# nyuolab/OmniBioTE

Hardware: AMD Instinct MI355X
Metric: MLM train tokens/sec, small (8L/1024d) ctx=1024 at 1/2/4/8 MI355X (higher is better)
Workload: dtype bf16

## Files before the change

omnibiote_amd/csrc/elementwise.hip:

```cpp
#include "common.h"
#include <stdlib.h>

namespace {

template <bool INVERSE>
__global__ __launch_bounds__(256) void rope_kernel(bf16* __restrict__ qkv, const float* __restrict__ cos_t,
                                                    const float* __restrict__ sin_t, int64_t rows, int64_t T, int C, int hs) {
    const int chunks_per_row = 2 * C / 8;
    const int64_t total = rows * chunks_per_row;
    for (int64_t i = (int64_t)blockIdx.x * blockDim.x + threadIdx.x; i < total; i += (int64_t)gridDim.x * blockDim.x) {
        const int64_t row = i / chunks_per_row;
        const int col = (int)(i % chunks_per_row) * 8;
        const int d = col % hs;
        const int64_t t = row % T;
        bf16* ptr = qkv + row * 3 * C + col;
        const bf16x8 v = *reinterpret_cast<const bf16x8*>(ptr);
        const f32x4 c = *reinterpret_cast<const f32x4*>(cos_t + t * (hs / 2) + d / 2);
        const f32x4 s = *reinterpret_cast<const f32x4*>(sin_t + t * (hs / 2) + d / 2);
        bf16x8 o;
#pragma unroll
        for (int j = 0; j < 4; ++j) {
            const float xe = bf2f(v[2 * j]), xo = bf2f(v[2 * j + 1]);
            const float sj = INVERSE ? -s[j] : s[j];
            o[2 * j] = f2bf(xe * c[j] - xo * sj);
            o[2 * j + 1] = f2bf(xe * sj + xo * c[j]);
        }
        *reinterpret_cast<bf16x8*>(ptr) = o;
    }
}

__device__ __forceinline__ int64_t clamp_tok(int64_t tok, int64_t vocab) { return tok < 0 ? 0 : (tok >= vocab ? vocab - 1 : tok); }

__global__ __launch_bounds__(256) void embed_fwd_kernel(const int64_t* __restrict__ idx, const bf16* __restrict__ wte,
                                                         bf16* __restrict__ out, int64_t rows, int cols, int64_t vocab, DropCfg dc) {
    const int cpr = cols / 8;
    const int64_t total = rows * cpr;
    for (int64_t i = (int64_t)blockIdx.x * blockDim.x + threadIdx.x; i < total; i += (int64_t)gridDim.x * blockDim.x) {
        const int64_t r = i / cpr;
        const int c = (int)(i % cpr) * 8;
        const int64_t tok = clamp_tok(idx[r], vocab);
        bf16x8 v = *reinterpret_cast<const bf16x8*>(wte + tok * cols + c);
        if (dc.thresh16) {
            const uint32_t rk = drop_rowkey((uint64_t)r, dc);
#pragma unroll
            for (int jj = 0; jj < 4; ++jj) {
                const uint32_t bits = drop_pair_bits(rk, (uint32_t)(c >> 1) + jj);
#pragma unroll
                for (int e = 0; e < 2; ++e) v[2 * jj + e] = drop_keep_bits(bits, (uint32_t)e, dc) ? f2bf(bf2f(v[2 * jj + e]) * dc.scale) : f2bf(0.f);
            }
        }
        *reinterpret_cast<bf16x8*>(out + r * cols + c) = v;
    }
}

__global__ __launch_bounds__(256) void dropout_kernel(const bf16* in, bf16* out, int64_t n8, int64_t cols, DropCfg dc) {
    for (int64_t i = (int64_t)blockIdx.x * blockDim.x + threadIdx.x; i < n8; i += (int64_t)gridDim.x * blockDim.x) {
        bf16x8 v = reinterpret_cast<const bf16x8*>(in)[i];
        const int64_t row = (i * 8) / cols;
        const uint32_t c = (uint32_t)((i * 8) - row * cols);
        const uint32_t rk = drop_rowkey((uint64_t)row, dc);
        for (int jj = 0; jj < 4; ++jj) {
            const uint32_t bits = drop_pair_bits(rk, (c >> 1) + jj);
#pragma unroll
            for (int e = 0; e < 2; ++e) v[2 * jj + e] = drop_keep_bits(bits, (uint32_t)e, dc) ? f2bf(bf2f(v[2 * jj + e]) * dc.scale) : f2bf(0.f);
        }
        reinterpret_cast<bf16x8*>(out)[i] = v;
    }
}

constexpr int EMB_CHUNK = 32;

template <bool ACC>
__device__ __forceinline__ void embed_store_row(bf16* dst, const float (&acc)[8]) {
    bf16x8 o;
#pragma unroll
    for (int j = 0; j < 8; ++j) o[j] = f2bf(acc[j]);
    if (ACC) {
        const bf16x8 old = *reinterpret_cast<const bf16x8*>(dst);
#pragma unroll
        for (int j = 0; j < 8; ++j) o[j] = f2bf(bf2f(old[j]) + bf2f(o[j]));
    }
    *reinterpret_cast<bf16x8*>(dst) = o;
}
template <bool ACC>
__device__ __forceinline__ void embed_store_row(float* dst, const float (&acc)[8]) {
    f32x4 lo = f32x4{acc[0], acc[1], acc[2], acc[3]}, hi = f32x4{acc[4], acc[5], acc[6], acc[7]};
    if (ACC) {
        lo += *reinterpret_cast<const f32x4*>(dst);
        hi += *reinterpret_cast<const f32x4*>(dst + 4);
    }
    *reinterpret_cast<f32x4*>(dst) = lo;
    *reinterpret_cast<f32x4*>(dst + 4) = hi;
}

template <bool ACC, class DST = bf16>
__global__ __launch_bounds__(128) void embed_bwd_chunk_kernel(const int64_t* __restrict__ idx, const int32_t* __restrict__ order,
                                                               const bf16* __restrict__ dout, DST* __restrict__ dwte,
                                                               float* __restrict__ slab, int64_t rows, int cols, int64_t vocab, DropCfg dc) {
    __shared__ int32_t s_row[EMB_CHUNK];
    __shared__ int64_t s_tok[EMB_CHUNK + 2];
    const int64_t c = blockIdx.x;
    const int64_t p0 = c * EMB_CHUNK;
    const int n = (int)((rows - p0) < EMB_CHUNK ? (rows - p0) : EMB_CHUNK);
    if (threadIdx.x < n) {
        const int32_t r = order[p0 + threadIdx.x];
        s_row[threadIdx.x] = r;
        s_tok[threadIdx.x + 1] = clamp_tok(idx[r], vocab);
    }
    if (threadIdx.x == 64) s_tok[0] = p0 > 0 ? clamp_tok(idx[order[p0 - 1]], vocab) : -1;
    if (threadIdx.x == 65) s_tok[n + 1] = (p0 + n < rows) ? clamp_tok(idx[order[p0 + n]], vocab) : -1;
    __syncthreads();
    const bool left_open = s_tok[0] == s_tok[1];
    const bool right_open = s_tok[n + 1] == s_tok[n];
    for (int col = threadIdx.x * 8; col < cols; col += 128 * 8) {
        float acc[8];
#pragma unroll
        for (int j = 0; j < 8; ++j) acc[j] = 0.f;
        int seg_start = 0;
        for (int i = 0; i < n; ++i) {
            const bf16x8 v = *reinterpret_cast<const bf16x8*>(dout + (int64_t)s_row[i] * cols + col);
            if (dc.thresh16) {
                const uint32_t rk = drop_rowkey((uint64_t)s_row[i], dc);
                for (int jj = 0; jj < 4; ++jj) {
                    const uint32_t bits = drop_pair_bits(rk, (uint32_t)(col >> 1) + jj);
#pragma unroll
                    for (int e = 0; e < 2; ++e)
                        if (drop_keep_bits(bits, (uint32_t)e, dc)) acc[2 * jj + e] += bf2f(f2bf(bf2f(v[2 * jj + e]) * dc.scale));
                }
            } else {
#pragma unroll
                for (int j = 0; j < 8; ++j) acc[j] += bf2f(v[j]);
            }
            const bool seg_end = (i == n - 1) || (s_tok[i + 2] != s_tok[i + 1]);
            if (seg_end) {
                const bool is_first = seg_start == 0, is_last = i == n - 1;
                if ((is_first && left_open) || (is_last && right_open)) {
                    float* dst = slab + ((c * 2 + (is_first ? 0 : 1)) * cols + col);
                    *reinterpret_cast<f32x4*>(dst) = f32x4{acc[0], acc[1], acc[2], acc[3]};
                    *reinterpret_cast<f32x4*>(dst + 4) = f32x4{acc[4], acc[5], acc[6], acc[7]};
                } else {
                    embed_store_row<ACC>(dwte + s_tok[i + 1] * cols + col, acc);
                }
#pragma unroll
                for (int j = 0; j < 8; ++j) acc[j] = 0.f;
                seg_start = i + 1;
            }
        }
    }
}

template <bool ACC, class DST = bf16>
__global__ __launch_bounds__(128) void embed_bwd_span_kernel(const int64_t* __restrict__ idx, const int32_t* __restrict__ order,
                                                              DST* __restrict__ dwte, const float* __restrict__ slab,
                                                              int64_t rows, int cols, int64_t nchunks, int64_t vocab) {
    const int64_t c = blockIdx.x;
    const int64_t p0 = c * EMB_CHUNK;
    const int64_t p1 = (p0 + EMB_CHUNK < rows) ? p0 + EMB_CHUNK : rows;
    const int64_t first = clamp_tok(idx[order[p0]], vocab), last = clamp_tok(idx[order[p1 - 1]], vocab);
    const bool single = first == last;
    const bool left_open = p0 > 0 && clamp_tok(idx[order[p0 - 1]], vocab) == first;
    const bool right_open = p1 < rows && clamp_tok(idx[order[p1]], vocab) == last;
    if (!right_open || (single && left_open)) return;
    const int slot0 = single ? 0 : 1;
    for (int col = threadIdx.x * 8; col < cols; col += 128 * 8) {
        float acc[8];
        const float* src = slab + ((c * 2 + slot0) * cols + col);
#pragma unroll
        for (int j = 0; j < 8; ++j) acc[j] = src[j];
        for (int64_t cc = c + 1; cc < nchunks; ++cc) {
            const int64_t q0 = cc * EMB_CHUNK;
            const int64_t q1 = (q0 + EMB_CHUNK < rows) ? q0 + EMB_CHUNK : rows;
            if (clamp_tok(idx[order[q0]], vocab) != last) break;
            const float* s2 = slab + ((cc * 2) * cols + col);
#pragma unroll
            for (int j = 0; j < 8; ++j) acc[j] += s2[j];
            if (clamp_tok(idx[order[q1 - 1]], vocab) != last) break;
        }
        embed_store_row<ACC>(dwte + last * cols + col, acc);
    }
}

__global__ __launch_bounds__(256) void acc32_add_kernel(float* __restrict__ acc32, const bf16* __restrict__ src, bf16* __restrict__ out,
                                                         int64_t n8, int mode) {
    for (int64_t i = (int64_t)blockIdx.x * 256 + threadIdx.x; i < n8; i += (int64_t)gridDim.x * 256) {
        float v[8];
        if (src) {
            const bf16x8 sv = *reinterpret_cast<const bf16x8*>(src + i * 8);
#pragma unroll
            for (int j = 0; j < 8; ++j) v[j] = bf2f(sv[j]);
        } else {
#pragma unroll
            for (int j = 0; j < 8; ++j) v[j] = 0.f;
        }
        if (mode != OBTE_ACC32_FIRST) {
            const f32x4 lo = *reinterpret_cast<const f32x4*>(acc32 + i * 8), hi = *reinterpret_cast<const f32x4*>(acc32 + i * 8 + 4);
#pragma unroll
            for (int j = 0; j < 4; ++j) { v[j] += lo[j]; v[4 + j] += hi[j]; }
        }
        if (src || mode == OBTE_ACC32_FIRST) {
            *reinterpret_cast<f32x4*>(acc32 + i * 8) = f32x4{v[0], v[1], v[2], v[3]};
            *reinterpret_cast<f32x4*>(acc32 + i * 8 + 4) = f32x4{v[4], v[5], v[6], v[7]};
        }
        if (mode == OBTE_ACC32_LAST) {
            bf16x8 o;
#pragma unroll
            for (int j = 0; j < 8; ++j) o[j] = f2bf(v[j]);
            *reinterpret_cast<bf16x8*>(out + i * 8) = o;
        }
    }
}

__global__ __launch_bounds__(256) void masked_ce_kernel(const bf16* __restrict__ logits, const int64_t* __restrict__ target,
                                                         const uint8_t* __restrict__ mlm_mask, const uint8_t* __restrict__ prev_mask,
                                                         const float* __restrict__ grad_scale, float row_scale,
                                                         float* __restrict__ row_loss, bf16* __restrict__ dlogits, int64_t vocab,
                                                         const int64_t* __restrict__ row_index, const float* __restrict__ row_scale_vec) {
    __shared__ float red[8];
    const int64_t r = blockIdx.x;
    const int64_t src = row_index ? row_index[r] : r;
    const int lane = threadIdx.x & 63, wave = threadIdx.x >> 6;
    bf16* drow = dlogits + r * vocab;
    if (!row_index && mlm_mask && !mlm_mask[r]) {
        if (threadIdx.x == 0 && row_loss) row_loss[r] = 0.f;
        if (prev_mask && !prev_mask[r]) return;
        const bf16x8 z = {};
        for (int64_t c = (int64_t)threadIdx.x * 8; c < vocab; c += 256 * 8) *reinterpret_cast<bf16x8*>(drow + c) = z;
        return;
    }
    const bf16* lrow = logits + src * vocab;
    float m = -INFINITY, l = 0.f;
    for (int64_t c = (int64_t)threadIdx.x * 8; c < vocab; c += 256 * 8) {
        const bf16x8 v = *reinterpret_cast<const bf16x8*>(lrow + c);
        float mx = bf2f(v[0]);
#pragma unroll
        for (int j = 1; j < 8; ++j) mx = fmaxf(mx, bf2f(v[j]));
        const float mn = fmaxf(m, mx);
        float add = 0.f;
#pragma unroll
        for (int j = 0; j < 8; ++j) add += __expf(bf2f(v[j]) - mn);
        l = l * __expf(m - mn) + add;
        m = mn;
    }
    const float wm = wave_max(m);
    l = wave_sum(m == -INFINITY ? 0.f : l * __expf(m - wm));
    if (lane == 0) { red[wave] = wm; red[4 + wave] = l; }
    __syncthreads();
    const float bm = fmaxf(fmaxf(red[0], red[1]), fmaxf(red[2], red[3]));
    const float bl = red[4] * __expf(red[0] - bm) + red[5] * __expf(red[1] - bm) + red[6] * __expf(red[2] - bm) + red[7] * __expf(red[3] - bm);
    const float lse = bm + __logf(bl);
    int64_t tgt = target[src];
    tgt = tgt < 0 ? 0 : (tgt >= vocab ? vocab - 1 : tgt);
    const float rsc = row_scale_vec ? row_scale * row_scale_vec[r] : row_scale;
    if (threadIdx.x == 0 && row_loss) row_loss[r] = (lse - bf2f(lrow[tgt])) * rsc;
    const float gs = grad_scale ? rsc * grad_scale[0] : rsc;
    for (int64_t c = (int64_t)threadIdx.x * 8; c < vocab; c += 256 * 8) {
        const bf16x8 v = *reinterpret_cast<const bf16x8*>(lrow + c);
        bf16x8 o;
#pragma unroll
        for (int j = 0; j < 8; ++j) {
            float p = __expf(bf2f(v[j]) - lse);
            if (c + j == tgt) p -= 1.0f;
            o[j] = f2bf(p * gs);
        }
        *reinterpret_cast<bf16x8*>(drow + c) = o;
    }
}

template <int NCH>
__global__ __launch_bounds__(256, 2) void masked_ce_regs_kernel(const bf16* __restrict__ logits, const int64_t* __restrict__ target,
                                                              const float* __restrict__ grad_scale, float row_scale,
                                                              float* __restrict__ row_loss, bf16* __restrict__ dlogits, int64_t vocab,
                                                              const int64_t* __restrict__ row_index, const float* __restrict__ row_scale_vec) {
    __shared__ float red[8];
    const int64_t r = blockIdx.x;
    const int64_t src = row_index ? row_index[r] : r;
    const int lane = threadIdx.x & 63, wave = threadIdx.x >> 6;
    bf16* drow = dlogits + r * vocab;
    const bf16* lrow = logits + src * vocab;
    bf16x8 v[NCH];
#pragma unroll
    for (int i = 0; i < NCH; ++i) {
        const int64_t c = ((int64_t)i * 256 + threadIdx.x) * 8;
        v[i] = bf16x8{};
        if (c < vocab) v[i] = *reinterpret_cast<const bf16x8*>(lrow + c);
    }
    float m = -INFINITY, l = 0.f;
#pragma unroll
    for (int i = 0; i < NCH; ++i) {
        const int64_t c = ((int64_t)i * 256 + threadIdx.x) * 8;
        if (c < vocab) {
            float mx = bf2f(v[i][0]);
#pragma unroll
            for (int j = 1; j < 8; ++j) mx = fmaxf(mx, bf2f(v[i][j]));
            const float mn = fmaxf(m, mx);
            float add = 0.f;
#pragma unroll
            for (int j = 0; j < 8; ++j) add += __expf(bf2f(v[i][j]) - mn);
            l = l * __expf(m - mn) + add;
            m = mn;
        }
    }
    const float wm = wave_max(m);
    l = wave_sum(m == -INFINITY ? 0.f : l * __expf(m - wm));
    if (lane == 0) { red[wave] = wm; red[4 + wave] = l; }
    __syncthreads();
    const float bm = fmaxf(fmaxf(red[0], red[1]), fmaxf(red[2], red[3]));
    const float bl = red[4] * __expf(red[0] - bm) + red[5] * __expf(red[1] - bm) + red[6] * __expf(red[2] - bm) + red[7] * __expf(red[3] - bm);
    const float lse = bm + __logf(bl);
    int64_t tgt = target[src];
    tgt = tgt < 0 ? 0 : (tgt >= vocab ? vocab - 1 : tgt);
    const float rsc = row_scale_vec ? row_scale * row_scale_vec[r] : row_scale;
    if (threadIdx.x == 0 && row_loss) row_loss[r] = (lse - bf2f(lrow[tgt])) * rsc;
    const float gs = grad_scale ? rsc * grad_scale[0] : rsc;
#pragma unroll
    for (int i = 0; i < NCH; ++i) {
        const int64_t c = ((int64_t)i * 256 + threadIdx.x) * 8;
        if (c < vocab) {
            bf16x8 o;
#pragma unroll
            for (int j = 0; j < 8; ++j) {
                float p = __expf(bf2f(v[i][j]) - lse);
                if (c + j == tgt) p -= 1.0f;
                o[j] = f2bf(p * gs);
            }
            *reinterpret_cast<bf16x8*>(drow + c) = o;
        }
    }
}

template <int NCH, bool NT>
__global__ __launch_bounds__(256, 1) void masked_ce_pipe_kernel(const bf16* __restrict__ logits, const int64_t* __restrict__ target,
                                                                 const float* __restrict__ grad_scale, float row_scale,
// ... 255 lines not shown
        }
        bf16x8 pp;
#pragma unroll
        for (int j = 0; j < 8; ++j) {
            const int h = j >> 2, k = j & 3;
            const float gj = bf2f(gg[j]) * cc;
            float pj = ww[h][k] * decay;
            const float m0 = mm[h][k];
            const float mj = __builtin_fmaf(w1, gj - m0, m0);
            float vj = vv[h][k] * b2;
            const float wg = w2 * gj;
            vj = __builtin_fmaf(wg, gj, vj);
            float d = sqrtf(vj);
            d = d / bc2s;
            d = d + eps;
            const float num = neg_step * mj;
            const float upd = num / d;
            pj = pj + upd;
            ww[h][k] = pj; mm[h][k] = mj; vv[h][k] = vj;
            pp[j] = f2bf(pj);
        }
        *reinterpret_cast<bf16x8*>(p + i) = pp;
#pragma unroll
        for (int h = 0; h < 2; ++h) {
            *reinterpret_cast<f32x4*>(w + i + 4 * h) = ww[h];
            *reinterpret_cast<f32x4*>(m + i + 4 * h) = mm[h];
            *reinterpret_cast<f32x4*>(v + i + 4 * h) = vv[h];
        }
    }
}

__global__ __launch_bounds__(256) void sumsq_multi_partials_kernel(MtTable t, float* __restrict__ partials) {
    __shared__ float red[4];
    const int ti = mt_find(t, blockIdx.x);
    const int64_t base = (int64_t)(blockIdx.x - t.first[ti]) * MT_CHUNK;
    const int64_t end = min(base + (int64_t)MT_CHUNK, t.n[ti]);
    const bf16* g = t.g[ti];
    float s = 0.f;
    for (int64_t i = base + threadIdx.x * 8; i < end; i += 256 * 8) {
        const bf16x8 v = *reinterpret_cast<const bf16x8*>(g + i);
#pragma unroll
        for (int j = 0; j < 8; ++j) { const float f = bf2f(v[j]); s += f * f; }
    }
    s = wave_sum(s);
    if ((threadIdx.x & 63) == 0) red[threadIdx.x >> 6] = s;
    __syncthreads();
    if (threadIdx.x == 0) partials[blockIdx.x] = ((red[0] + red[1]) + red[2]) + red[3];
}

__global__ __launch_bounds__(256) void clip_coef_kernel(const float* __restrict__ partials, int64_t n, float max_norm, float* __restrict__ out) {
    __shared__ double red[256];
    double s = 0.0;
    for (int64_t i = threadIdx.x; i < n; i += 256) s += (double)partials[i];
    red[threadIdx.x] = s;
    __syncthreads();
#pragma unroll
    for (int o = 128; o > 0; o >>= 1) {
        if ((int)threadIdx.x < o) red[threadIdx.x] += red[threadIdx.x + o];
        __syncthreads();
    }
    if (threadIdx.x == 0) {
        const float norm_sq = (float)red[0];
        out[0] = norm_sq;
        out[1] = fminf(1.0f, (1.0f / (sqrtf(norm_sq) + 1e-6f)) * max_norm);
    }
}

inline unsigned stream_grid(int64_t work_items, int per_block) {
    int64_t b = cdiv64(work_items, per_block);
    return (unsigned)(b < 1 ? 1 : (b > 2048 ? 2048 : b));
}

}

extern "C" int obte_rope_qk_inplace(obte_bf16* qkv, const float* cos_t, const float* sin_t, int64_t B, int64_t T,
                                    int n_head, int head_dim, int inverse, obte_stream s) {
    OBTE_REQUIRE(qkv && cos_t && sin_t, "obte_rope_qk_inplace: null pointer");
    OBTE_REQUIRE_ALIGNED("obte_rope_qk_inplace", qkv, "qkv", 16);
    OBTE_REQUIRE_ALIGNED("obte_rope_qk_inplace", cos_t, "cos_t", 16);
    OBTE_REQUIRE_ALIGNED("obte_rope_qk_inplace", sin_t, "sin_t", 16);
    OBTE_REQUIRE(B > 0 && T > 0 && n_head > 0 && head_dim % 8 == 0, "obte_rope_qk_inplace: head_dim must be a multiple of 8");
    const int C = n_head * head_dim;
    const int64_t rows = B * T, total = rows * (2 * C / 8);
    hipStream_t st = (hipStream_t)s;
    if (inverse)
        hipLaunchKernelGGL((rope_kernel<true>), dim3(stream_grid(total, 256)), dim3(256), 0, st, (bf16*)qkv, cos_t, sin_t, rows, T, C, head_dim);
    else
        hipLaunchKernelGGL((rope_kernel<false>), dim3(stream_grid(total, 256)), dim3(256), 0, st, (bf16*)qkv, cos_t, sin_t, rows, T, C, head_dim);
    OBTE_CHECK_LAUNCH("obte_rope_qk_inplace");
    return OBTE_OK;
}

static int check_p(const char* who, float p) {
    OBTE_REQUIRE(p >= 0.f && p < 1.f, "%s: dropout p must be in [0, 1) (got %g)", who, (double)p);
    return OBTE_OK;
}

extern "C" int obte_embedding_fwd_dropout(const int64_t* idx, const obte_bf16* wte, obte_bf16* out, int64_t rows, int cols,
                                          int64_t vocab, float p, uint64_t seed, obte_stream s) {
    OBTE_REQUIRE(idx && wte && out, "obte_embedding_fwd: null pointer");
    OBTE_REQUIRE_ALIGNED("obte_embedding_fwd", wte, "wte", 16);
    OBTE_REQUIRE_ALIGNED("obte_embedding_fwd", out, "out", 16);
    OBTE_REQUIRE(rows >= 0 && cols > 0 && cols % 8 == 0 && vocab > 0, "obte_embedding_fwd: cols must be a multiple of 8");
    if (check_p("obte_embedding_fwd", p)) return OBTE_EINVAL;
    if (rows == 0) return OBTE_OK;
    hipLaunchKernelGGL(embed_fwd_kernel, dim3(stream_grid(rows * (cols / 8), 256)), dim3(256), 0, (hipStream_t)s, idx,
                       (const bf16*)wte, (bf16*)out, rows, cols, vocab, make_drop(p, seed, OBTE_SITE_EMBED));
    OBTE_CHECK_LAUNCH("obte_embedding_fwd");
    return OBTE_OK;
}

extern "C" int obte_embedding_fwd(const int64_t* idx, const obte_bf16* wte, obte_bf16* out, int64_t rows, int cols,
                                  int64_t vocab, obte_stream s) {
    return obte_embedding_fwd_dropout(idx, wte, out, rows, cols, vocab, 0.f, 0, s);
}

__global__ __launch_bounds__(256) void dropout_rows_kernel(const bf16* __restrict__ in, const bf16* __restrict__ aux, bf16* __restrict__ out,
                                                           const int64_t* __restrict__ rows, int64_t n_rows, int cols, DropCfg cfg) {
    const int64_t i = (int64_t)blockIdx.x * 4 + (threadIdx.x >> 6);
    if (i >= n_rows) return;
    const int lane = threadIdx.x & 63;
    const uint32_t rk = drop_rowkey((uint64_t)rows[i], cfg);
    for (int c = lane * 8; c < cols; c += 512) {
        bf16x8 v = *reinterpret_cast<const bf16x8*>(in + i * cols + c);
        bf16x8 a = {};
        if (aux) a = *reinterpret_cast<const bf16x8*>(aux + i * cols + c);
#pragma unroll
        for (int jj = 0; jj < 4; ++jj) {
            const uint32_t bits = drop_pair_bits(rk, ((uint32_t)c >> 1) + jj);
#pragma unroll
            for (int e = 0; e < 2; ++e) {
                const int j = 2 * jj + e;
                const float t = drop_keep_bits(bits, (uint32_t)e, cfg) ? bf2f(f2bf(bf2f(v[j]) * cfg.scale)) : 0.f;
                v[j] = aux ? f2bf(bf2f(a[j]) + t) : f2bf(t);
            }
        }
        *reinterpret_cast<bf16x8*>(out + i * cols + c) = v;
    }
}

extern "C" int obte_dropout_bf16(const obte_bf16* in, obte_bf16* out, int64_t n, int64_t cols, float p, uint64_t seed, int32_t site,
                                 obte_stream s) {
    OBTE_REQUIRE_ALIGNED("obte_dropout_bf16", in, "in", 16);
    OBTE_REQUIRE_ALIGNED("obte_dropout_bf16", out, "out", 16);
    OBTE_REQUIRE(in && out && n > 0 && n % 8 == 0, "obte_dropout_bf16: null pointer or n not a positive multiple of 8");
    OBTE_REQUIRE(cols > 0 && cols % 8 == 0 && n % cols == 0 && cols < (1ll << 32), "obte_dropout_bf16: cols must be a multiple of 8 that divides n");
    if (check_p("obte_dropout_bf16", p)) return OBTE_EINVAL;
    hipLaunchKernelGGL(dropout_kernel, dim3(stream_grid(n / 8, 256)), dim3(256), 0, (hipStream_t)s, (const bf16*)in, (bf16*)out, n / 8,
                       cols, make_drop(p, seed, (uint32_t)site));
    OBTE_CHECK_LAUNCH("obte_dropout_bf16");
    return OBTE_OK;
}

extern "C" int64_t obte_embedding_bwd_ws_bytes(int64_t rows, int cols) {
    return cdiv64(rows, EMB_CHUNK) * 2 * (int64_t)cols * (int64_t)sizeof(float);
}

extern "C" int obte_embedding_bwd_dropout(const int64_t* idx, const int32_t* order, const obte_bf16* dout, obte_bf16* dwte,
                                          void* ws, int64_t rows, int cols, int64_t vocab, int accumulate, float p, uint64_t seed,
                                          obte_stream s) {
    OBTE_REQUIRE(idx && order && dout && dwte && ws, "obte_embedding_bwd: null pointer");
    OBTE_REQUIRE_ALIGNED("obte_embedding_bwd", dout, "dout", 16);
    OBTE_REQUIRE_ALIGNED("obte_embedding_bwd", dwte, "dwte", 16);
    OBTE_REQUIRE_ALIGNED("obte_embedding_bwd", ws, "ws", 16);
    if (check_p("obte_embedding_bwd", p)) return OBTE_EINVAL;
    const DropCfg dc = make_drop(p, seed, OBTE_SITE_EMBED);
    OBTE_REQUIRE(rows > 0 && cols > 0 && cols % 8 == 0 && vocab > 0, "obte_embedding_bwd: bad shape");
    OBTE_REQUIRE(rows < (1ll << 31), "obte_embedding_bwd: too many rows");
    hipStream_t st = (hipStream_t)s;
    if (!accumulate && hipMemsetAsync(dwte, 0, (size_t)vocab * cols * sizeof(obte_bf16), st) != hipSuccess) {
        obte_set_error("obte_embedding_bwd: memset failed");
        return OBTE_ELAUNCH;
    }
    const int64_t nchunks = cdiv64(rows, EMB_CHUNK);
    if (accumulate)
        hipLaunchKernelGGL(embed_bwd_chunk_kernel<true>, dim3((unsigned)nchunks), dim3(128), 0, st, idx, order, (const bf16*)dout,
                           (bf16*)dwte, (float*)ws, rows, cols, vocab, dc);
    else
        hipLaunchKernelGGL(embed_bwd_chunk_kernel<false>, dim3((unsigned)nchunks), dim3(128), 0, st, idx, order, (const bf16*)dout,
                           (bf16*)dwte, (float*)ws, rows, cols, vocab, dc);
    OBTE_CHECK_LAUNCH("obte_embedding_bwd(chunk)");
    if (accumulate)
        hipLaunchKernelGGL(embed_bwd_span_kernel<true>, dim3((unsigned)nchunks), dim3(128), 0, st, idx, order, (bf16*)dwte,
                           (const float*)ws, rows, cols, nchunks, vocab);
    else
        hipLaunchKernelGGL(embed_bwd_span_kernel<false>, dim3((unsigned)nchunks), dim3(128), 0, st, idx, order, (bf16*)dwte,
                           (const float*)ws, rows, cols, nchunks, vocab);
    OBTE_CHECK_LAUNCH("obte_embedding_bwd(span)");
    return OBTE_OK;
}

extern "C" int obte_acc32_add_bf16(float* acc32, const obte_bf16* src, obte_bf16* out, int64_t n, int mode, obte_stream s) {
    OBTE_REQUIRE_ALIGNED("obte_acc32_add_bf16", acc32, "acc32", 16);
    OBTE_REQUIRE_ALIGNED("obte_acc32_add_bf16", src, "src", 16);
    OBTE_REQUIRE_ALIGNED("obte_acc32_add_bf16", out, "out", 16);
    OBTE_REQUIRE(acc32 && n > 0 && n % 8 == 0, "obte_acc32_add_bf16: null buffer or n not a positive multiple of 8");
    OBTE_REQUIRE(mode >= OBTE_ACC32_FIRST && mode <= OBTE_ACC32_LAST && (mode != OBTE_ACC32_LAST || out), "obte_acc32_add_bf16: bad mode, or LAST without out");
    if (!src && mode == OBTE_ACC32_MORE) return OBTE_OK;
    hipLaunchKernelGGL(acc32_add_kernel, dim3(stream_grid(n / 8, 256)), dim3(256), 0, (hipStream_t)s, acc32, (const bf16*)src, (bf16*)out, n / 8, mode);
    OBTE_CHECK_LAUNCH("obte_acc32_add_bf16");
    return OBTE_OK;
}

extern "C" int obte_embedding_bwd_acc32(const int64_t* idx, const int32_t* order, const obte_bf16* dout, float* acc32, obte_bf16* dwte,
                                        void* ws, int64_t rows, int cols, int64_t vocab, int mode, float p, uint64_t seed, obte_stream s) {
    OBTE_REQUIRE(idx && order && dout && acc32 && ws, "obte_embedding_bwd_acc32: null pointer");
    OBTE_REQUIRE_ALIGNED("obte_embedding_bwd_acc32", dout, "dout", 16);
    OBTE_REQUIRE_ALIGNED("obte_embedding_bwd_acc32", acc32, "acc32", 16);
    OBTE_REQUIRE_ALIGNED("obte_embedding_bwd_acc32", dwte, "dwte", 16);
    OBTE_REQUIRE_ALIGNED("obte_embedding_bwd_acc32", ws, "ws", 16);
    OBTE_REQUIRE(mode >= OBTE_ACC32_FIRST && mode <= OBTE_ACC32_LAST && (mode != OBTE_ACC32_LAST || dwte), "obte_embedding_bwd_acc32: bad mode, or LAST without dwte");
    if (check_p("obte_embedding_bwd_acc32", p)) return OBTE_EINVAL;
    const DropCfg dc = make_drop(p, seed, OBTE_SITE_EMBED);
    OBTE_REQUIRE(rows > 0 && cols > 0 && cols % 8 == 0 && vocab > 0, "obte_embedding_bwd_acc32: bad shape");
    OBTE_REQUIRE(rows < (1ll << 31), "obte_embedding_bwd_acc32: too many rows");
    hipStream_t st = (hipStream_t)s;
    const bool first = mode == OBTE_ACC32_FIRST;
    if (first && hipMemsetAsync(acc32, 0, (size_t)vocab * cols * sizeof(float), st) != hipSuccess) {
        obte_set_error("obte_embedding_bwd_acc32: memset failed");
        return OBTE_ELAUNCH;
    }
    const int64_t nchunks = cdiv64(rows, EMB_CHUNK);
    if (first)
        hipLaunchKernelGGL((embed_bwd_chunk_kernel<false, float>), dim3((unsigned)nchunks), dim3(128), 0, st, idx, order, (const bf16*)dout, acc32, (float*)ws,
                           rows, cols, vocab, dc);
    else
        hipLaunchKernelGGL((embed_bwd_chunk_kernel<true, float>), dim3((unsigned)nchunks), dim3(128), 0, st, idx, order, (const bf16*)dout, acc32, (float*)ws,
                           rows, cols, vocab, dc);
    OBTE_CHECK_LAUNCH("obte_embedding_bwd_acc32(chunk)");
    if (first)
        hipLaunchKernelGGL((embed_bwd_span_kernel<false, float>), dim3((unsigned)nchunks), dim3(128), 0, st, idx, order, acc32, (const float*)ws, rows, cols,
                           nchunks, vocab);
    else
        hipLaunchKernelGGL((embed_bwd_span_kernel<true, float>), dim3((unsigned)nchunks), dim3(128), 0, st, idx, order, acc32, (const float*)ws, rows, cols,
                           nchunks, vocab);
    OBTE_CHECK_LAUNCH("obte_embedding_bwd_acc32(span)");
    if (mode == OBTE_ACC32_LAST) return obte_acc32_add_bf16(acc32, nullptr, dwte, vocab * (int64_t)cols, OBTE_ACC32_LAST, s);
    return OBTE_OK;
}

extern "C" int obte_embedding_bwd_acc(const int64_t* idx, const int32_t* order, const obte_bf16* dout, obte_bf16* dwte,
                                      void* ws, int64_t rows, int cols, int64_t vocab, int accumulate, obte_stream s) {
    return obte_embedding_bwd_dropout(idx, order, dout, dwte, ws, rows, cols, vocab, accumulate, 0.f, 0, s);
}

extern "C" int obte_embedding_bwd(const int64_t* idx, const int32_t* order, const obte_bf16* dout, obte_bf16* dwte,
                                  void* ws, int64_t rows, int cols, int64_t vocab, obte_stream s) {
    return obte_embedding_bwd_dropout(idx, order, dout, dwte, ws, rows, cols, vocab, 0, 0.f, 0, s);
}

extern "C" int obte_masked_ce_fwd_bwd_reuse(const obte_bf16* logits, const int64_t* target, const uint8_t* mlm_mask,
                                            const uint8_t* prev_mask, const float* grad_scale, float row_scale, float* row_loss,
                                            obte_bf16* dlogits, int64_t rows, int64_t vocab, obte_stream s) {
    OBTE_REQUIRE(logits && target && mlm_mask && grad_scale && dlogits, "obte_masked_ce_fwd_bwd: null pointer");
    OBTE_REQUIRE_ALIGNED("obte_masked_ce_fwd_bwd", logits, "logits", 16);
    OBTE_REQUIRE_ALIGNED("obte_masked_ce_fwd_bwd", dlogits, "dlogits", 16);
    OBTE_REQUIRE(rows > 0 && rows < (1ll << 31) && vocab > 0 && vocab % 8 == 0, "obte_masked_ce_fwd_bwd: vocab must be a multiple of 8");
    hipLaunchKernelGGL(masked_ce_kernel, dim3((unsigned)rows), dim3(256), 0, (hipStream_t)s, (const bf16*)logits, target, mlm_mask,
                       prev_mask, grad_scale, row_scale, row_loss, (bf16*)dlogits, vocab, (const int64_t*)nullptr, (const float*)nullptr);
    OBTE_CHECK_LAUNCH("obte_masked_ce_fwd_bwd");
    return OBTE_OK;
}

namespace {
__global__ __launch_bounds__(256) void rows_copy_kernel(const bf16* __restrict__ src, const int64_t* __restrict__ rows, bf16* __restrict__ dst,
                                                         int64_t n_rows, int64_t total_rows, int cols, int scatter) {
    const int wave = threadIdx.x >> 6, lane = threadIdx.x & 63;
    const int64_t i = (int64_t)blockIdx.x * 4 + wave;
    if (i >= n_rows) return;
    int64_t r = rows[i];
    r = r < 0 ? 0 : (r >= total_rows ? total_rows - 1 : r);
    const bf16* s = src + (scatter ? i : r) * cols;
    bf16* d = dst + (scatter ? r : i) * cols;
    for (int c = lane * 8; c < cols; c += 64 * 8) *reinterpret_cast<bf16x8*>(d + c) = *reinterpret_cast<const bf16x8*>(s + c);
}
}
extern "C" int obte_rows_gather_bf16(const obte_bf16* src, const int64_t* rows, obte_bf16* dst, int64_t n_rows, int64_t total_rows, int32_t cols, obte_stream s) {
    OBTE_REQUIRE(src && rows && dst, "obte_rows_gather_bf16: null pointer");
    OBTE_REQUIRE_ALIGNED("obte_rows_gather_bf16", src, "src", 16);
    OBTE_REQUIRE_ALIGNED("obte_rows_gather_bf16", dst, "dst", 16);
    OBTE_REQUIRE(n_rows > 0 && total_rows > 0 && cols > 0 && cols % 8 == 0, "obte_rows_gather_bf16: need n_rows, total_rows > 0 and cols %% 8 == 0");
    hipLaunchKernelGGL(rows_copy_kernel, dim3((unsigned)cdiv64(n_rows, 4)), dim3(256), 0, (hipStream_t)s, (const bf16*)src, rows, (bf16*)dst, n_rows, total_rows, cols, 0);
    OBTE_CHECK_LAUNCH("obte_rows_gather_bf16");
    return OBTE_OK;
}
extern "C" int obte_rows_scatter_bf16(const obte_bf16* src, const int64_t* rows, obte_bf16* dst, int64_t n_rows, int64_t total_rows, int32_t cols, obte_stream s) {
    OBTE_REQUIRE(src && rows && dst, "obte_rows_scatter_bf16: null pointer");
    OBTE_REQUIRE_ALIGNED("obte_rows_scatter_bf16", src, "src", 16);
    OBTE_REQUIRE_ALIGNED("obte_rows_scatter_bf16", dst, "dst", 16);
    OBTE_REQUIRE(n_rows > 0 && n_rows <= total_rows && cols > 0 && cols % 8 == 0, "obte_rows_scatter_bf16: need 0 < n_rows <= total_rows and cols %% 8 == 0");
    if (hipMemsetAsync(dst, 0, (size_t)total_rows * cols * 2, (hipStream_t)s) != hipSuccess) { obte_set_error("obte_rows_scatter_bf16: memset failed"); return OBTE_ELAUNCH; }
    hipLaunchKernelGGL(rows_copy_kernel, dim3((unsigned)cdiv64(n_rows, 4)), dim3(256), 0, (hipStream_t)s, (const bf16*)src, rows, (bf16*)dst, n_rows, total_rows, cols, 1);
    OBTE_CHECK_LAUNCH("obte_rows_scatter_bf16");
    return OBTE_OK;
}

extern "C" int obte_masked_ce_rows(const obte_bf16* logits, const int64_t* target, const int64_t* row_index, const float* grad_scale,
                                   float row_scale, const float* row_scale_vec, float* row_loss, obte_bf16* dlogits_rows, int64_t n_rows,
                                   int64_t total_rows, int64_t vocab, obte_stream s) {
    OBTE_REQUIRE(logits && target && dlogits_rows && row_loss, "obte_masked_ce_rows: null pointer");
    OBTE_REQUIRE_ALIGNED("obte_masked_ce_rows", logits, "logits", 16);
    OBTE_REQUIRE_ALIGNED("obte_masked_ce_rows", dlogits_rows, "dlogits_rows", 16);
    OBTE_REQUIRE(n_rows > 0 && n_rows <= total_rows && total_rows < (1ll << 31) && vocab > 0 && vocab % 8 == 0,
                 "obte_masked_ce_rows: need 0 < n_rows <= total_rows and vocab %% 8 == 0");
    OBTE_REQUIRE(row_index || n_rows == total_rows, "obte_masked_ce_rows: without a row list, logits and target hold exactly the n_rows listed rows");
    OBTE_REQUIRE((const void*)logits != (const void*)dlogits_rows, "obte_masked_ce_rows: dlogits_rows must not alias logits");
    const int prof = obte_prof_begin((hipStream_t)s, 112, n_rows, vocab, 1);
    struct CeCfg { int regs_on, pipe_on, nt_on, pipe_grid; };
    static const CeCfg cfg = [] {
        CeCfg c;
        const char* e = getenv("OBTE_CE_REGS"); c.regs_on = (e && e[0] == '0') ? 0 : 1;
        e = getenv("OBTE_CE_PIPE"); c.pipe_on = (e && e[0] == '0') ? 0 : 1;
        e = getenv("OBTE_CE_NT"); c.nt_on = (e && e[0] == '1') ? 1 : 0;
        e = getenv("OBTE_CE_GRID"); c.pipe_grid = e ? atoi(e) : 256;
        if (c.pipe_grid < 1 || c.pipe_grid > 4096) c.pipe_grid = 256;
        return c;
    }();
    const int regs_on = cfg.regs_on, pipe_on = cfg.pipe_on, nt_on = cfg.nt_on, pipe_grid = cfg.pipe_grid;
    if (regs_on && pipe_on && vocab == 256 * 32 * 8 && n_rows > pipe_grid) {
        const dim3 grid((unsigned)pipe_grid);
        const int smem = (int)(vocab * 2 + 128);
        if (nt_on) {
            (void)hipFuncSetAttribute((const void*)masked_ce_pipe_kernel<32, true>, hipFuncAttributeMaxDynamicSharedMemorySize, smem);
            hipLaunchKernelGGL((masked_ce_pipe_kernel<32, true>), grid, dim3(256), smem, (hipStream_t)s, (const bf16*)logits, target, grad_scale, row_scale,
                               row_loss, (bf16*)dlogits_rows, n_rows, row_index, row_scale_vec);
        } else {
            (void)hipFuncSetAttribute((const void*)masked_ce_pipe_kernel<32, false>, hipFuncAttributeMaxDynamicSharedMemorySize, smem);
            hipLaunchKernelGGL((masked_ce_pipe_kernel<32, false>), grid, dim3(256), smem, (hipStream_t)s, (const bf16*)logits, target, grad_scale, row_scale,
                               row_loss, (bf16*)dlogits_rows, n_rows, row_index, row_scale_vec);
        }
    } else if (regs_on && vocab <= 256 * 8 * 8)
        hipLaunchKernelGGL((masked_ce_regs_kernel<8>), dim3((unsigned)n_rows), dim3(256), 0, (hipStream_t)s, (const bf16*)logits, target,
                           grad_scale, row_scale, row_loss, (bf16*)dlogits_rows, vocab, row_index, row_scale_vec);
    else if (regs_on && vocab <= 256 * 32 * 8)
        hipLaunchKernelGGL((masked_ce_regs_kernel<32>), dim3((unsigned)n_rows), dim3(256), 0, (hipStream_t)s, (const bf16*)logits, target,
                           grad_scale, row_scale, row_loss, (bf16*)dlogits_rows, vocab, row_index, row_scale_vec);
    else
        hipLaunchKernelGGL(masked_ce_kernel, dim3((unsigned)n_rows), dim3(256), 0, (hipStream_t)s, (const bf16*)logits, target,
                           (const uint8_t*)nullptr, (const uint8_t*)nullptr, grad_scale, row_scale, row_loss, (bf16*)dlogits_rows, vocab, row_index,
                           row_scale_vec);
    obte_prof_end(prof, (hipStream_t)s);
    OBTE_CHECK_LAUNCH("obte_masked_ce_rows");
    return OBTE_OK;
}

extern "C" int obte_masked_ce_fwd_bwd(const obte_bf16* logits, const int64_t* target, const uint8_t* mlm_mask,
                                      const float* grad_scale, float row_scale, float* loss_sum, float* row_loss,
                                      obte_bf16* dlogits, int64_t rows, int64_t vocab, obte_stream s) {
    (void)loss_sum;
    return obte_masked_ce_fwd_bwd_reuse(logits, target, mlm_mask, nullptr, grad_scale, row_scale, row_loss, dlogits, rows, vocab, s);
}

extern "C" int obte_adamw_bf16(obte_bf16* p, const obte_bf16* g, obte_bf16* m, obte_bf16* v, int64_t n, float lr,
                               float beta1, float beta2, float eps, float weight_decay, int32_t step,
                               const float* clip_coef, obte_stream s) {
    OBTE_REQUIRE(p && g && m && v, "obte_adamw_bf16: null pointer");
    OBTE_REQUIRE_ALIGNED("obte_adamw_bf16", p, "p", 16);
    OBTE_REQUIRE_ALIGNED("obte_adamw_bf16", g, "g", 16);
    OBTE_REQUIRE_ALIGNED("obte_adamw_bf16", m, "m", 16);
    OBTE_REQUIRE_ALIGNED("obte_adamw_bf16", v, "v", 16);
    OBTE_REQUIRE(n > 0 && n % 8 == 0 && step >= 1, "obte_adamw_bf16: n must be a positive multiple of 8, step >= 1");
    const float bc1 = 1.0f - powf(beta1, (float)step);
    const float bc2s = sqrtf(1.0f - powf(beta2, (float)step));
    hipLaunchKernelGGL(adamw_kernel, dim3(stream_grid(n / 8, 256)), dim3(256), 0, (hipStream_t)s, (bf16*)p, (const bf16*)g,
                       (bf16*)m, (bf16*)v, n / 8, lr, beta1, beta2, eps, weight_decay, bc1, bc2s, clip_coef);
    OBTE_CHECK_LAUNCH("obte_adamw_bf16");
    return OBTE_OK;
}

extern "C" int obte_sumsq_bf16(const obte_bf16* g, int64_t n, float* out, obte_stream s) {
    OBTE_REQUIRE(g && out, "obte_sumsq_bf16: null pointer");
    OBTE_REQUIRE_ALIGNED("obte_sumsq_bf16", g, "g", 16);
    OBTE_REQUIRE(n > 0 && n % 8 == 0, "obte_sumsq_bf16: n must be a positive multiple of 8");
    hipLaunchKernelGGL(sumsq_kernel, dim3(stream_grid(n / 8, 256)), dim3(256), 0, (hipStream_t)s, (const bf16*)g, n / 8, out);
    OBTE_CHECK_LAUNCH("obte_sumsq_bf16");
    return OBTE_OK;
}

extern "C" int obte_adamw_multi_bf16(const obte_mt_args* a, float beta1, float beta2, float eps, const float* clip_coef, obte_stream s) {
    MtTable t;
    const int blocks = mt_build(a, beta1, beta2, &t, "obte_adamw_multi_bf16", true);
    if (blocks < 0) return blocks;
    hipLaunchKernelGGL(adamw_multi_kernel, dim3(blocks), dim3(256), 0, (hipStream_t)s, t, beta1, beta2, eps, clip_coef);
    OBTE_CHECK_LAUNCH("obte_adamw_multi_bf16");
    return OBTE_OK;
}

extern "C" int obte_adamw_multi_bf16_ref(const obte_mt_args* a, double beta1, double beta2, double eps, const float* clip_coef, obte_stream s) {
// ... 153 lines not shown
```

Baseline: 1.293 million.

## Batch embedding-backward loads and parallelize span reduction with chunk-end tokens

The chunk kernel now loads dout rows and the old dwte values in groups of eight so the memory requests overlap. It also writes each chunk's first and last token into a small ends array. The span kernel reads those ends instead of re-gathering idx[order[...]]. It finds where a run stops using wavefront ballots, then splits the columns across a 2D grid of 64-thread blocks with batched slab loads. The aim is to cut serialized dependent gathers and latency in the embedding-gradient scatter. The cost is extra workspace and more register pressure.

```diff
diff --git a/omnibiote_amd/csrc/elementwise.hip b/omnibiote_amd/csrc/elementwise.hip
--- a/omnibiote_amd/csrc/elementwise.hip
+++ b/omnibiote_amd/csrc/elementwise.hip
@@ -69,34 +69,67 @@
 }
 
 constexpr int EMB_CHUNK = 32;
+constexpr int EMB_GROUP = 8;
+constexpr int EMB_SPAN_COLS = 256;
+constexpr int EMB_SPAN_GROUP = 32;
+
+typedef __attribute__((ext_vector_type(2))) int64_t emb_i64x2;
+
+template <class DST, int N> struct emb_old;
+template <> struct emb_old<bf16, 8> { bf16x8 v; };
+template <> struct emb_old<bf16, 4> { bf16x4 v; };
+template <> struct emb_old<float, 8> { f32x4 lo, hi; };
+template <> struct emb_old<float, 4> { f32x4 lo; };
+__device__ __forceinline__ void embed_load_old(const bf16* src, emb_old<bf16, 8>& o) { o.v = *reinterpret_cast<const bf16x8*>(src); }
+__device__ __forceinline__ void embed_load_old(const bf16* src, emb_old<bf16, 4>& o) { o.v = *reinterpret_cast<const bf16x4*>(src); }
+__device__ __forceinline__ void embed_load_old(const float* src, emb_old<float, 8>& o) {
+    o.lo = *reinterpret_cast<const f32x4*>(src);
+    o.hi = *reinterpret_cast<const f32x4*>(src + 4);
+}
+__device__ __forceinline__ void embed_load_old(const float* src, emb_old<float, 4>& o) { o.lo = *reinterpret_cast<const f32x4*>(src); }
 
 template <bool ACC>
-__device__ __forceinline__ void embed_store_row(bf16* dst, const float (&acc)[8]) {
+__device__ __forceinline__ void embed_store_row(bf16* dst, const float (&acc)[8], const emb_old<bf16, 8>& old) {
     bf16x8 o;
 #pragma unroll
     for (int j = 0; j < 8; ++j) o[j] = f2bf(acc[j]);
     if (ACC) {
-        const bf16x8 old = *reinterpret_cast<const bf16x8*>(dst);
-#pragma unroll
-        for (int j = 0; j < 8; ++j) o[j] = f2bf(bf2f(old[j]) + bf2f(o[j]));
+#pragma unroll
+        for (int j = 0; j < 8; ++j) o[j] = f2bf(bf2f(old.v[j]) + bf2f(o[j]));
     }
     *reinterpret_cast<bf16x8*>(dst) = o;
 }
 template <bool ACC>
-__device__ __forceinline__ void embed_store_row(float* dst, const float (&acc)[8]) {
+__device__ __forceinline__ void embed_store_row(float* dst, const float (&acc)[8], const emb_old<float, 8>& old) {
     f32x4 lo = f32x4{acc[0], acc[1], acc[2], acc[3]}, hi = f32x4{acc[4], acc[5], acc[6], acc[7]};
     if (ACC) {
-        lo += *reinterpret_cast<const f32x4*>(dst);
-        hi += *reinterpret_cast<const f32x4*>(dst + 4);
+        lo += old.lo;
+        hi += old.hi;
     }
     *reinterpret_cast<f32x4*>(dst) = lo;
     *reinterpret_cast<f32x4*>(dst + 4) = hi;
+}
+template <bool ACC>
+__device__ __forceinline__ void embed_store_quad(bf16* dst, const f32x4& acc, const emb_old<bf16, 4>& old) {
+    bf16x4 o;
+#pragma unroll
+    for (int j = 0; j < 4; ++j) o[j] = f2bf(acc[j]);
+    if (ACC) {
+#pragma unroll
+        for (int j = 0; j < 4; ++j) o[j] = f2bf(bf2f(old.v[j]) + bf2f(o[j]));
+    }
+    *reinterpret_cast<bf16x4*>(dst) = o;
+}
+template <bool ACC>
+__device__ __forceinline__ void embed_store_quad(float* dst, const f32x4& acc, const emb_old<float, 4>& old) {
+    *reinterpret_cast<f32x4*>(dst) = ACC ? acc + old.lo : acc;
 }
 
 template <bool ACC, class DST = bf16>
 __global__ __launch_bounds__(128) void embed_bwd_chunk_kernel(const int64_t* __restrict__ idx, const int32_t* __restrict__ order,
                                                                const bf16* __restrict__ dout, DST* __restrict__ dwte,
-                                                               float* __restrict__ slab, int64_t rows, int cols, int64_t vocab, DropCfg dc) {
+                                                               float* __restrict__ slab, int64_t* __restrict__ ends, int64_t rows, int cols,
+                                                               int64_t vocab, DropCfg dc) {
     __shared__ int32_t s_row[EMB_CHUNK];
     __shared__ int64_t s_tok[EMB_CHUNK + 2];
     const int64_t c = blockIdx.x;
@@ -110,6 +143,10 @@
     if (threadIdx.x == 64) s_tok[0] = p0 > 0 ? clamp_tok(idx[order[p0 - 1]], vocab) : -1;
     if (threadIdx.x == 65) s_tok[n + 1] = (p0 + n < rows) ? clamp_tok(idx[order[p0 + n]], vocab) : -1;
     __syncthreads();
+    if (threadIdx.x == 0) {
+        ends[2 * c] = s_tok[1];
+        ends[2 * c + 1] = s_tok[n];
+    }
     const bool left_open = s_tok[0] == s_tok[1];
     const bool right_open = s_tok[n + 1] == s_tok[n];
     for (int col = threadIdx.x * 8; col < cols; col += 128 * 8) {
@@ -117,67 +154,109 @@
 #pragma unroll
         for (int j = 0; j < 8; ++j) acc[j] = 0.f;
         int seg_start = 0;
-        for (int i = 0; i < n; ++i) {
-            const bf16x8 v = *reinterpret_cast<const bf16x8*>(dout + (int64_t)s_row[i] * cols + col);
-            if (dc.thresh16) {
-                const uint32_t rk = drop_rowkey((uint64_t)s_row[i], dc);
-                for (int jj = 0; jj < 4; ++jj) {
-                    const uint32_t bits = drop_pair_bits(rk, (uint32_t)(col >> 1) + jj);
-#pragma unroll
-                    for (int e = 0; e < 2; ++e)
-                        if (drop_keep_bits(bits, (uint32_t)e, dc)) acc[2 * jj + e] += bf2f(f2bf(bf2f(v[2 * jj + e]) * dc.scale));
+#pragma unroll 1
+        for (int g = 0; g < n; g += EMB_GROUP) {
+            bf16x8 v[EMB_GROUP];
+            emb_old<DST, 8> old[EMB_GROUP];
+#pragma unroll
+            for (int k = 0; k < EMB_GROUP; ++k) {
+                const int ii = g + k < n ? g + k : n - 1;
+                v[k] = *reinterpret_cast<const bf16x8*>(dout + (int64_t)s_row[ii] * cols + col);
+                if (ACC) embed_load_old(dwte + s_tok[ii + 1] * cols + col, old[k]);
+            }
+#pragma unroll
+            for (int k = 0; k < EMB_GROUP; ++k) {
+                const int i = g + k;
+                if (i >= n) break;
+                if (dc.thresh16) {
+                    const uint32_t rk = drop_rowkey((uint64_t)s_row[i], dc);
+                    for (int jj = 0; jj < 4; ++jj) {
+                        const uint32_t bits = drop_pair_bits(rk, (uint32_t)(col >> 1) + jj);
+#pragma unroll
+                        for (int e = 0; e < 2; ++e)
+                            if (drop_keep_bits(bits, (uint32_t)e, dc)) acc[2 * jj + e] += bf2f(f2bf(bf2f(v[k][2 * jj + e]) * dc.scale));
+                    }
+                } else {
+#pragma unroll
+                    for (int j = 0; j < 8; ++j) acc[j] += bf2f(v[k][j]);
                 }
-            } else {
-#pragma unroll
-                for (int j = 0; j < 8; ++j) acc[j] += bf2f(v[j]);
+                const bool seg_end = (i == n - 1) || (s_tok[i + 2] != s_tok[i + 1]);
+                if (seg_end) {
+                    const bool is_first = seg_start == 0, is_last = i == n - 1;
+                    if ((is_first && left_open) || (is_last && right_open)) {
+                        float* dst = slab + ((c * 2 + (is_first ? 0 : 1)) * cols + col);
+                        *reinterpret_cast<f32x4*>(dst) = f32x4{acc[0], acc[1], acc[2], acc[3]};
+                        *reinterpret_cast<f32x4*>(dst + 4) = f32x4{acc[4], acc[5], acc[6], acc[7]};
+                    } else {
+                        embed_store_row<ACC>(dwte + s_tok[i + 1] * cols + col, acc, old[k]);
+                    }
+#pragma unroll
+                    for (int j = 0; j < 8; ++j) acc[j] = 0.f;
+                    seg_start = i + 1;
+                }
             }
-            const bool seg_end = (i == n - 1) || (s_tok[i + 2] != s_tok[i + 1]);
-            if (seg_end) {
-                const bool is_first = seg_start == 0, is_last = i == n - 1;
-                if ((is_first && left_open) || (is_last && right_open)) {
-                    float* dst = slab + ((c * 2 + (is_first ? 0 : 1)) * cols + col);
-                    *reinterpret_cast<f32x4*>(dst) = f32x4{acc[0], acc[1], acc[2], acc[3]};
-                    *reinterpret_cast<f32x4*>(dst + 4) = f32x4{acc[4], acc[5], acc[6], acc[7]};
-                } else {
-                    embed_store_row<ACC>(dwte + s_tok[i + 1] * cols + col, acc);
-                }
-#pragma unroll
-                for (int j = 0; j < 8; ++j) acc[j] = 0.f;
-                seg_start = i + 1;
-            }
         }
     }
 }
 
 template <bool ACC, class DST = bf16>
-__global__ __launch_bounds__(128) void embed_bwd_span_kernel(const int64_t* __restrict__ idx, const int32_t* __restrict__ order,
-                                                              DST* __restrict__ dwte, const float* __restrict__ slab,
-                                                              int64_t rows, int cols, int64_t nchunks, int64_t vocab) {
+__global__ __launch_bounds__(64) void embed_bwd_span_kernel(const int64_t* __restrict__ ends, DST* __restrict__ dwte,
+                                                             const float* __restrict__ slab, int cols, int64_t nchunks) {
     const int64_t c = blockIdx.x;
-    const int64_t p0 = c * EMB_CHUNK;
-    const int64_t p1 = (p0 + EMB_CHUNK < rows) ? p0 + EMB_CHUNK : rows;
-    const int64_t first = clamp_tok(idx[order[p0]], vocab), last = clamp_tok(idx[order[p1 - 1]], vocab);
+    const int64_t first = ends[2 * c], last = ends[2 * c + 1];
+    const int64_t before = ends[c > 0 ? 2 * c - 1 : 0], after = ends[c + 1 < nchunks ? 2 * c + 2 : 2 * c + 1];
     const bool single = first == last;
-    const bool left_open = p0 > 0 && clamp_tok(idx[order[p0 - 1]], vocab) == first;
-    const bool right_open = p1 < rows && clamp_tok(idx[order[p1]], vocab) == last;
+    const bool left_open = c > 0 && before == first;
+    const bool right_open = c + 1 < nchunks && after == last;
     if (!right_open || (single && left_open)) return;
-    const int slot0 = single ? 0 : 1;
-    for (int col = threadIdx.x * 8; col < cols; col += 128 * 8) {
-        float acc[8];
-        const float* src = slab + ((c * 2 + slot0) * cols + col);
-#pragma unroll
-        for (int j = 0; j < 8; ++j) acc[j] = src[j];
-        for (int64_t cc = c + 1; cc < nchunks; ++cc) {
-            const int64_t q0 = cc * EMB_CHUNK;
-            const int64_t q1 = (q0 + EMB_CHUNK < rows) ? q0 + EMB_CHUNK : rows;
-            if (clamp_tok(idx[order[q0]], vocab) != last) break;
-            const float* s2 = slab + ((cc * 2) * cols + col);
-#pragma unroll
-            for (int j = 0; j < 8; ++j) acc[j] += s2[j];
-            if (clamp_tok(idx[order[q1 - 1]], vocab) != last) break;
-        }
-        embed_store_row<ACC>(dwte + last * cols + col, acc);
-    }
+    int64_t stop = c + 1;
+    for (;;) {
+        emb_i64x2 e[2];
+        unsigned long long not_head[2], not_tail[2];
+#pragma unroll
+        for (int h = 0; h < 2; ++h) {
+            const int64_t cc = stop + 64 * h + threadIdx.x;
+            e[h] = *reinterpret_cast<const emb_i64x2*>(ends + 2 * (cc < nchunks ? cc : nchunks - 1));
+        }
+#pragma unroll
+        for (int h = 0; h < 2; ++h) {
+            const bool head = stop + 64 * h + threadIdx.x < nchunks && e[h][0] == last;
+            not_head[h] = __ballot(!head);
+            not_tail[h] = __ballot(head && e[h][1] != last);
+        }
+        const int h = (not_head[0] | not_tail[0]) ? 0 : 1;
+        if (not_head[h] | not_tail[h]) {
+            const int fh = not_head[h] ? __builtin_ctzll(not_head[h]) : 64, ft = not_tail[h] ? __builtin_ctzll(not_tail[h]) : 64;
+            stop += 64 * h + (fh < ft ? fh : ft + 1);
+            break;
+        }
+        stop += 128;
+    }
+    const int col = blockIdx.y * EMB_SPAN_COLS + threadIdx.x * 4;
+    if (col >= cols) return;
+    DST* dst = dwte + last * cols + col;
+    emb_old<DST, 4> old;
+    if (ACC) embed_load_old(dst, old);
+    f32x4 acc = *reinterpret_cast<const f32x4*>(slab + ((c * 2 + (single ? 0 : 1)) * cols + col));
+#pragma unroll 1
+    for (int64_t cc = c + 1; cc < stop; cc += EMB_SPAN_GROUP) {
+        f32x4 part[EMB_SPAN_GROUP];
+#pragma unroll
+        for (int k = 0; k < EMB_SPAN_GROUP; ++k) {
+            const int64_t ci = cc + k < stop ? cc + k : stop - 1;
+            part[k] = *reinterpret_cast<const f32x4*>(slab + (ci * 2 * cols + col));
+        }
+        __builtin_amdgcn_sched_barrier(0);
+        if (cc + EMB_SPAN_GROUP <= stop) {
+#pragma unroll
+            for (int k = 0; k < EMB_SPAN_GROUP; ++k) acc += part[k];
+        } else {
+#pragma unroll
+            for (int k = 0; k < EMB_SPAN_GROUP; ++k)
+                if (cc + k < stop) acc += part[k];
+        }
+    }
+    embed_store_quad<ACC>(dst, acc, old);
 }
 
 __global__ __launch_bounds__(256) void acc32_add_kernel(float* __restrict__ acc32, const bf16* __restrict__ src, bf16* __restrict__ out,
@@ -739,8 +818,10 @@
     return OBTE_OK;
 }
 
+static int64_t embed_slab_bytes(int64_t rows, int cols) { return cdiv64(rows, EMB_CHUNK) * 2 * (int64_t)cols * (int64_t)sizeof(float); }
+
 extern "C" int64_t obte_embedding_bwd_ws_bytes(int64_t rows, int cols) {
-    return cdiv64(rows, EMB_CHUNK) * 2 * (int64_t)cols * (int64_t)sizeof(float);
+    return embed_slab_bytes(rows, cols) + cdiv64(rows, EMB_CHUNK) * 2 * (int64_t)sizeof(int64_t);
 }
 
 extern "C" int obte_embedding_bwd_dropout(const int64_t* idx, const int32_t* order, const obte_bf16* dout, obte_bf16* dwte,
@@ -760,19 +841,19 @@
         return OBTE_ELAUNCH;
     }
     const int64_t nchunks = cdiv64(rows, EMB_CHUNK);
+    int64_t* ends = (int64_t*)((char*)ws + embed_slab_bytes(rows, cols));
+    const dim3 span_grid((unsigned)nchunks, (unsigned)((cols + EMB_SPAN_COLS - 1) / EMB_SPAN_COLS));
     if (accumulate)
         hipLaunchKernelGGL(embed_bwd_chunk_kernel<true>, dim3((unsigned)nchunks), dim3(128), 0, st, idx, order, (const bf16*)dout,
-                           (bf16*)dwte, (float*)ws, rows, cols, vocab, dc);
+                           (bf16*)dwte, (float*)ws, ends, rows, cols, vocab, dc);
     else
         hipLaunchKernelGGL(embed_bwd_chunk_kernel<false>, dim3((unsigned)nchunks), dim3(128), 0, st, idx, order, (const bf16*)dout,
-                           (bf16*)dwte, (float*)ws, rows, cols, vocab, dc);
+                           (bf16*)dwte, (float*)ws, ends, rows, cols, vocab, dc);
     OBTE_CHECK_LAUNCH("obte_embedding_bwd(chunk)");
     if (accumulate)
-        hipLaunchKernelGGL(embed_bwd_span_kernel<true>, dim3((unsigned)nchunks), dim3(128), 0, st, idx, order, (bf16*)dwte,
-                           (const float*)ws, rows, cols, nchunks, vocab);
+        hipLaunchKernelGGL(embed_bwd_span_kernel<true>, span_grid, dim3(64), 0, st, (const int64_t*)ends, (bf16*)dwte, (const float*)ws, cols, nchunks);
     else
-        hipLaunchKernelGGL(embed_bwd_span_kernel<false>, dim3((unsigned)nchunks), dim3(128), 0, st, idx, order, (bf16*)dwte,
-                           (const float*)ws, rows, cols, nchunks, vocab);
+        hipLaunchKernelGGL(embed_bwd_span_kernel<false>, span_grid, dim3(64), 0, st, (const int64_t*)ends, (bf16*)dwte, (const float*)ws, cols, nchunks);
     OBTE_CHECK_LAUNCH("obte_embedding_bwd(span)");
     return OBTE_OK;
 }
@@ -808,19 +889,19 @@
         return OBTE_ELAUNCH;
     }
     const int64_t nchunks = cdiv64(rows, EMB_CHUNK);
+    int64_t* ends = (int64_t*)((char*)ws + embed_slab_bytes(rows, cols));
+    const dim3 span_grid((unsigned)nchunks, (unsigned)((cols + EMB_SPAN_COLS - 1) / EMB_SPAN_COLS));
     if (first)
         hipLaunchKernelGGL((embed_bwd_chunk_kernel<false, float>), dim3((unsigned)nchunks), dim3(128), 0, st, idx, order, (const bf16*)dout, acc32, (float*)ws,
-                           rows, cols, vocab, dc);
+                           ends, rows, cols, vocab, dc);
     else
         hipLaunchKernelGGL((embed_bwd_chunk_kernel<true, float>), dim3((unsigned)nchunks), dim3(128), 0, st, idx, order, (const bf16*)dout, acc32, (float*)ws,
-                           rows, cols, vocab, dc);
+                           ends, rows, cols, vocab, dc);
     OBTE_CHECK_LAUNCH("obte_embedding_bwd_acc32(chunk)");
     if (first)
-        hipLaunchKernelGGL((embed_bwd_span_kernel<false, float>), dim3((unsigned)nchunks), dim3(128), 0, st, idx, order, acc32, (const float*)ws, rows, cols,
-                           nchunks, vocab);
+        hipLaunchKernelGGL((embed_bwd_span_kernel<false, float>), span_grid, dim3(64), 0, st, (const int64_t*)ends, acc32, (const float*)ws, cols, nchunks);
     else
-        hipLaunchKernelGGL((embed_bwd_span_kernel<true, float>), dim3((unsigned)nchunks), dim3(128), 0, st, idx, order, acc32, (const float*)ws, rows, cols,
-                           nchunks, vocab);
+        hipLaunchKernelGGL((embed_bwd_span_kernel<true, float>), span_grid, dim3(64), 0, st, (const int64_t*)ends, acc32, (const float*)ws, cols, nchunks);
     OBTE_CHECK_LAUNCH("obte_embedding_bwd_acc32(span)");
     if (mode == OBTE_ACC32_LAST) return obte_acc32_add_bf16(acc32, nullptr, dwte, vocab * (int64_t)cols, OBTE_ACC32_LAST, s);
     return OBTE_OK;
```

Result: no change. 1.296 million (median of 6 runs) (+0.2%).
